# eBay/Sequence-Semantic-Embedding

Measured on AMD Instinct MI355X. Metric: encoded seqs/sec (+ query x target cosine-scores/sec, top-1 vs ref), higher is better.
Workload: dtype f32; 1 GPU; configs[1]: classification stand-in, dual-encoder LSTM H=S=256 E=50 T=32 V=32000; encode 16384 source seqs/GPU/step + cosine top-10 vs 571-target index; batch_per_gpu=16384, seq_len=32, targets=571, parallelism=dp1, weights=random-init (reference initialisers, seed 0)

## Files before the change

### sequence-semantic-embedding_amd/csrc/score_topk.hip

```cpp
#include <cstdlib>

#include "sse_kernels.h"

#define SC_THREADS 512
#define SC_KC 16
#ifndef SC_PRIO_K
#define SC_PRIO_K 1
#define SC_PRIO_E 0
#endif

#ifdef SSE_SCORE_CLOCK
#include <cstdio>
__device__ long long g_score_clk[8 * 8];
#define SC_CLK_DECL long long ck_[8] = {0, 0, 0, 0, 0, 0, 0, 0}, ck_t = clock64();
#define SC_CLK(i)                   \
  {                                 \
    const long long n_ = clock64(); \
    ck_[i] += n_ - ck_t;            \
    ck_t = n_;                      \
  }
#else
#define SC_CLK_DECL
#define SC_CLK(i)
#endif
// ... 786 lines not shown
  hipLaunchKernelGGL(frag32_to_bf16_kernel, dim3((int)(blocks < 16384 ? blocks : 16384)), dim3(256), 0, stream,
                     reinterpret_cast<const f32x4 *>(idxp), NT, KG, KG16, total8, reinterpret_cast<f32x4 *>(out));
  return hipGetLastError();
}

__device__ __forceinline__ int si_key(float f) {
  const int i = __float_as_int(f);
  return i >= 0 ? i : (i ^ 0x7FFFFFFF);
}
__device__ __forceinline__ float si_val(int k) { return __int_as_float(k >= 0 ? k : (k ^ 0x7FFFFFFF)); }
template <int CTRL, int ROWMASK>
__device__ __forceinline__ float dpp_f(float x) {
  return __int_as_float(__builtin_amdgcn_update_dpp(__float_as_int(x), __float_as_int(x), CTRL, ROWMASK, 0xF, false));
}
__device__ __forceinline__ float wave_max_f(float x) {
  x = fmaxf(x, dpp_f<0x128, 0xF>(x));
  x = fmaxf(x, dpp_f<0x124, 0xF>(x));
  x = fmaxf(x, dpp_f<0x122, 0xF>(x));
  x = fmaxf(x, dpp_f<0x121, 0xF>(x));
  x = fmaxf(x, dpp_f<0x142, 0xA>(x));
  x = fmaxf(x, dpp_f<0x143, 0xC>(x));
  return __int_as_float(__builtin_amdgcn_readlane(__float_as_int(x), 63));
}
template <int JMAX>
#ifdef SSE_SCORE_CLOCK
#define SI_CLK_PARAMS , long long (&ck_)[8], long long &ck_t
#define SI_CLK_ARGS , ck_, ck_t
#else
#define SI_CLK_PARAMS
#define SI_CLK_ARGS
#endif
__device__ __forceinline__ void si_select4(const SmallIndexArgs &a, const float *sc, int NP, int NT, int qt, int q0, int lane SI_CLK_PARAMS) {
  constexpr int QW = 4;
  const int J = (NT * 32 + 63) / 64;
  float v[QW][JMAX];
#pragma unroll
  for (int j = 0; j < JMAX; ++j) {
    const int row = lane + 64 * j;
#pragma unroll
    for (int c = 0; c < QW; ++c) v[c][j] = (j < J && row < NT * 32) ? sc[(q0 + c) * NP + row] : NEG_INF;
  }
  int lok[QW], hik[QW];
  float lm[QW];
  bool done[QW];
#pragma unroll
  for (int c = 0; c < QW; ++c) {
    float m = NEG_INF;
#pragma unroll
    for (int j = 0; j < JMAX; ++j) m = fmaxf(m, v[c][j]);
    lm[c] = m;
    lok[c] = si_key(-wave_max_f(-m));
    hik[c] = si_key(wave_max_f(m)) + 1;
    done[c] = false;
  }
  SC_CLK(5)
// ... 23 lines not shown
      int cr = -1, base = 0;
#pragma unroll
      for (int j = 0; j < JMAX; ++j) {
        const bool take = (j < J) & (v[c][j] >= T) & (v[c][j] > NEG_INF);
        const unsigned long long mask = __ballot(take);
        const int n = __popcll(mask);
        const int slot = base + (int)__builtin_amdgcn_mbcnt_hi((unsigned)(mask >> 32), __builtin_amdgcn_mbcnt_lo((unsigned)mask, 0u));
        const int dst = (take && slot < 63) ? slot : 63;
        const int gs = __builtin_amdgcn_ds_permute(dst * 4, __float_as_int(v[c][j]));
        const int gr = __builtin_amdgcn_ds_permute(dst * 4, lane + 64 * j);
        const bool recv = (lane >= base) & (lane < base + n) & (lane < 63);
        cs = recv ? __int_as_float(gs) : cs;
        cr = recv ? gr : cr;
        base += n;
      }
      const int nw = base < 63 ? base : 63;
      int rank = 0;
      for (int l = 0; l < nw; ++l) {
        const float os = __int_as_float(__builtin_amdgcn_readlane(__float_as_int(cs), l));
        const int orow = __builtin_amdgcn_readlane(cr, l);
        rank += ((os > cs) | ((os == cs) & (orow < cr))) ? 1 : 0;
      }
      const bool mine = lane < nw;
      if (mine && rank < SC_KC) {
        a.part_scores[(size_t)query * SC_KC + rank] = cs;
        a.part_ids[(size_t)query * SC_KC + rank] = cr;
      }
      if (lane >= nw && lane < SC_KC) {
        a.part_scores[(size_t)query * SC_KC + lane] = NEG_INF;
        a.part_ids[(size_t)query * SC_KC + lane] = -1;
      }
      const unsigned long long m16 = __ballot(mine && rank == SC_KC - 1);
      const float last = m16 ? __int_as_float(__builtin_amdgcn_readlane(__float_as_int(cs), __ffsll((long long)m16) - 1)) : NEG_INF;
      if (lane == 0) a.part_bnd[query] = (base > 63) ? __builtin_inff() : last;
    }
  }
}

template <int KGC>
__global__ __launch_bounds__(256) void score_small_index_kernel(SmallIndexArgs a) {
  extern __shared__ __attribute__((aligned(16))) float si_sc[];
  const int tid = threadIdx.x, lane = tid & 63, w = __builtin_amdgcn_readfirstlane(tid >> 6);
  const int NT = a.NT, NP = NT * 32 + 1;
  const int qt = blockIdx.x;
  float *sc = si_sc;
  SC_CLK_DECL
  f32x4 b[KGC];
  {
    const int row = qt * 32 + (lane & 31), kb = (lane >> 5) * 4;
    const float *src = a.q_rows + (size_t)(row < a.Q ? row : 0) * a.S + kb;
    const bool vec = (a.S & 3) == 0 && (reinterpret_cast<uintptr_t>(a.q_rows) & 15) == 0 && KGC * 8 <= a.S;
#pragma unroll
    for (int kg = 0; kg < KGC; ++kg) {
      f32x4 v = {0, 0, 0, 0};
      if (vec) {
        v = *reinterpret_cast<const f32x4 *>(src + kg * 8);
      } else {
#pragma unroll
        for (int e = 0; e < 4; ++e)
          if (kg * 8 + kb + e < a.S) v[e] = src[kg * 8 + e];
      }
      if (row >= a.Q) v = f32x4{0, 0, 0, 0};
      b[kg] = v;
    }
  }
  SC_CLK(0)
  for (int t = w; t < NT; t += 4) {
    const f32x4 *ap = reinterpret_cast<const f32x4 *>(a.idxp) + (size_t)t * KGC * 64 + lane;
    f32x16 acc = {0, 0, 0, 0, 0, 0, 0, 0, 0, 0, 0, 0, 0, 0, 0, 0};
    f32x4 ar[4];
#pragma unroll
    for (int d = 0; d < 4; ++d) ar[d] = ap[(d < KGC ? d : 0) * 64];
#pragma unroll
    for (int kg = 0; kg < KGC; ++kg) {
      __builtin_amdgcn_sched_barrier(0);
#pragma unroll
      for (int e = 0; e < 4; ++e) acc = __builtin_amdgcn_mfma_f32_32x32x2f32(ar[kg & 3][e], b[kg][e], acc, 0, 0, 0);
      __builtin_amdgcn_sched_barrier(0);
      ar[kg & 3] = ap[(kg + 4 < KGC ? kg + 4 : kg) * 64];
    }
    const int rb = t * 32 + 4 * (lane >> 5);
    float *col = sc + (lane & 31) * NP;
#pragma unroll
    for (int r = 0; r < 16; ++r) {
      const int row = rb + (r & 3) + 8 * (r >> 2);
      col[row] = (row < a.N) ? acc[r] : NEG_INF;
    }
  }
  SC_CLK(1)
  __syncthreads();
  SC_CLK(2)
  if (NT * 32 <= 640) {
    si_select4<10>(a, sc, NP, NT, qt, w * 8, lane SI_CLK_ARGS);
    SC_CLK(3)
    si_select4<10>(a, sc, NP, NT, qt, w * 8 + 4, lane SI_CLK_ARGS);
    SC_CLK(4)
#ifdef SSE_SCORE_CLOCK
    if (blockIdx.x == gridDim.x / 2 && lane == 0)
      for (int i = 0; i < 8; ++i) g_score_clk[w * 8 + i] = ck_[i];
#endif
  } else {
    si_select4<16>(a, sc, NP, NT, qt, w * 8, lane SI_CLK_ARGS);
    si_select4<16>(a, sc, NP, NT, qt, w * 8 + 4, lane SI_CLK_ARGS);
  }
}
bool score_small_index_applies(int Q, int KG, int64_t NT) {
  return Q >= 1024 && (KG == 32 || KG == 8 || KG == 7) && NT * 32 <= 1024 && (size_t)32 * (NT * 32 + 1) * sizeof(float) <= (size_t)144 * 1024;
}
hipError_t launch_score_small_index(const SmallIndexArgs &a, hipStream_t stream) {
  if (!score_small_index_applies(a.Q, a.KG, a.NT)) return hipErrorInvalidValue;
  const size_t lds = (size_t)32 * (a.NT * 32 + 1) * sizeof(float);
  const dim3 grid((a.Q + 31) / 32), block(256);
  auto go = [&](auto kernel) -> hipError_t {
    hipError_t e = hipFuncSetAttribute(reinterpret_cast<const void *>(kernel), hipFuncAttributeMaxDynamicSharedMemorySize, (int)lds);
    if (e != hipSuccess) return e;
    hipLaunchKernelGGL(kernel, grid, block, lds, stream, a);
    return hipGetLastError();
  };
  if (a.KG == 8) return go(score_small_index_kernel<8>);
  if (a.KG == 7) return go(score_small_index_kernel<7>);
  const hipError_t e32 = go(score_small_index_kernel<32>);
  if (e32 != hipSuccess) return e32;
#ifdef SSE_SCORE_CLOCK
  if (a.Q >= 8192) {
    static int n = 0;
    if (n++ % 8 == 3) {
      long long v[64];
      (void)hipStreamSynchronize(stream);
      (void)hipMemcpyFromSymbol(v, HIP_SYMBOL(g_score_clk), sizeof v);
      for (int w = 0; w < 4; w += 3)
        fprintf(stderr, "[small index clock Q=%d NT=%d] wave %d cycles: query fragments %lld | scores (MFMA + LDS stores) %lld | barrier %lld | selection: loads + bounds %lld | bisection %lld | winners + rank + stores %lld (both batches)\n",
                a.Q, a.NT, w, v[w * 8 + 0], v[w * 8 + 1], v[w * 8 + 2], v[w * 8 + 5], v[w * 8 + 6], v[w * 8 + 3] + v[w * 8 + 4]);
    }
  }
#endif
  return hipGetLastError();
}

hipError_t launch_score_topk(const ScoreArgs &a_in, hipStream_t stream) {
  ScoreArgs a = a_in;
#ifdef SSE_SCORE_MEASURE
  {
    static const int dbg = getenv("SSE_SCORE_DBG") ? atoi(getenv("SSE_SCORE_DBG")) : 0;
    a.dbg = dbg;
// ... 305 lines not shown
      a.cert[qo] = ok ? 1 : 0;
      if (a.col_thr) a.col_thr[qo] = ok ? __builtin_inff() : __double2float_rd(t - (double)(a.eps32 * qnorm));
      if (a.col_slot) {
        a.col_slot[qo] = ok ? -1 : qo;
        a.col_cnt[qo] = 0;
      }
      if (a.host_flag) {
        a.host_cert[qo] = ok ? 1 : 0;
        if (qo == 0 && a.host_err) *a.host_err = a.err_in ? *a.err_in : 0;
        __hip_atomic_store(a.host_flag + qo, a.seq, __ATOMIC_RELEASE, __HIP_MEMORY_SCOPE_SYSTEM);
      }
    }
  }
}

#ifndef RS_NB
#define RS_NB 4
#endif
__device__ __forceinline__ double readlane_f64(double v, int l) {
  const long long b = __double_as_longlong(v);
  const int lo = __builtin_amdgcn_readlane((int)b, l), hi = __builtin_amdgcn_readlane((int)(b >> 32), l);
  return __longlong_as_double(((long long)hi << 32) | (unsigned int)lo);
}
__global__ __launch_bounds__(256) void rescore_small_kernel(RescoreArgs a) {
  const int lane = threadIdx.x & 63;
  const int q = blockIdx.x * 4 + (threadIdx.x >> 6);
  if (q >= a.Q) return;
  if (a.q_count && q >= *a.q_count) return;
  const int qo = a.qmap ? a.qmap[q] : q;
  const float *qrow = a.q + (size_t)q * a.S;
  const int KG = (a.S + 7) / 8;
#ifdef SSE_SCORE_CLOCK
  long long rk_[6] = {0, 0, 0, 0, 0, 0}, rk_t = clock64();
#define RS_CLK(i) { const long long n_ = clock64(); rk_[i] += n_ - rk_t; rk_t = n_; }
#else
#define RS_CLK(i)
#endif
  const bool have = lane < a.NC;
  const int id = have ? a.part_ids[(size_t)q * a.NC + lane] : -1;
  const float sc = have ? a.part_scores[(size_t)q * a.NC + lane] : NEG_INF;
  const float bnd = (lane < a.NC / SC_KC) ? a.part_bnd[(size_t)q * (a.NC / SC_KC) + lane] : NEG_INF;
  double qn = 0.0;
  for (int d = lane; d < a.S; d += 64) qn += (double)qrow[d] * qrow[d];
#pragma unroll
  for (int o = 32; o > 0; o >>= 1) qn += __shfl_xor(qn, o);
  const float qnorm = (float)sqrt(qn);
  const float eps_q = a.eps * qnorm;
  RS_CLK(0)

  unsigned u = __float_as_uint(sc);
  u = (u & 0x80000000u) ? ~u : (u | 0x80000000u);
  const unsigned long long key = (id < 0) ? 0ull : (((unsigned long long)u << 32) | (unsigned long long)(0xFFFFFFFFu - (unsigned)id));
  const int key_lo = (int)(unsigned)key, key_hi = (int)(unsigned)(key >> 32);
  int rank = 0;
  for (int j = 0; j < a.NC; ++j) {
    const unsigned long long kj = ((unsigned long long)(unsigned)__builtin_amdgcn_readlane(key_hi, j) << 32) |
                                  (unsigned long long)(unsigned)__builtin_amdgcn_readlane(key_lo, j);
    rank += (kj > key) ? 1 : 0;
  }
  const unsigned long long kmask = __ballot(key != 0ull && rank == a.k - 1);
  const float kth = kmask ? __int_as_float(__builtin_amdgcn_readlane(__float_as_int(sc), __ffsll((long long)kmask) - 1)) : NEG_INF;
  const bool in_win = (id >= 0) && (sc >= kth - 2.0f * eps_q);
  float mmax = NEG_INF;
  for (int j = 0; j < a.NC / SC_KC; ++j) mmax = fmaxf(mmax, __int_as_float(__builtin_amdgcn_readlane(__float_as_int(bnd), j)));
  const unsigned long long wmask = __ballot(in_win);
  const int nwin = __popcll(wmask);
  const int mi = __popcll(wmask & ((1ull << lane) - 1ull));
  const int idm = __builtin_amdgcn_ds_permute((in_win ? mi : 63) * 4, id);
  RS_CLK(1)
  double exm = -__builtin_inf();
  for (int m0 = 0; m0 < nwin; m0 += RS_NB) {
    int64_t n[RS_NB];
#pragma unroll
    for (int c = 0; c < RS_NB; ++c) n[c] = __builtin_amdgcn_readlane(idm, (m0 + c < nwin) ? m0 + c : 0);
    const double tot = wave_exact_dot_packed<RS_NB>(qrow, a.idx32, a.idx64, n, a.S, KG, lane, a.idx_rm);
    const int want = lane - m0;
    const double got = __shfl(tot, packed_lane_of_value<RS_NB>(want & (RS_NB - 1)));
    if (want >= 0 && want < RS_NB && lane < nwin) exm = got;
  }
  RS_CLK(2)
  int r2 = 0;
  for (int j = 0; j < nwin; ++j)
    r2 += before(readlane_f64(exm, j), (int64_t)__builtin_amdgcn_readlane(idm, j), exm, (int64_t)idm) ? 1 : 0;
  const bool member = lane < nwin;
  if (member && r2 < a.k) {
    a.out_scores[(size_t)qo * a.k + r2] = exm;
    a.out_ids[(size_t)qo * a.k + r2] = a.id_base + idm;
    if (a.host_flag) {
      a.host_scores[(size_t)qo * a.k + r2] = exm;
      a.host_ids[(size_t)qo * a.k + r2] = a.id_base + idm;
    }
  }
  const unsigned long long tmask = __ballot(member && r2 == a.k - 1);
  const double theta = tmask ? readlane_f64(exm, __ffsll((long long)tmask) - 1) : -__builtin_inf();
  if (a.host_flag) __threadfence_system();
  RS_CLK(3)
#ifdef SSE_SCORE_CLOCK
  if (q == a.Q / 2 && lane == 0) {
    rk_[4] = nwin;
    for (int i = 0; i < 6; ++i) g_score_clk[i] = rk_[i];
  }
#endif
  if (lane == 0) {
    const bool ok = (nwin >= a.k) && ((double)mmax + (double)eps_q < theta);
    a.cert[qo] = ok ? 1 : 0;
    if (a.col_thr) a.col_thr[qo] = ok ? __builtin_inff() : __double2float_rd(theta - (double)(a.eps32 * qnorm));
    if (a.col_slot) {
      a.col_slot[qo] = ok ? -1 : qo;
      a.col_cnt[qo] = 0;
    }
    if (a.host_flag) {
      a.host_cert[qo] = ok ? 1 : 0;
      if (qo == 0 && a.host_err) *a.host_err = a.err_in ? *a.err_in : 0;
      __hip_atomic_store(a.host_flag + qo, a.seq, __ATOMIC_RELEASE, __HIP_MEMORY_SCOPE_SYSTEM);
    }
  }
}

hipError_t launch_rescore(const RescoreArgs &a, hipStream_t stream) {
  if (a.NC > RS_MAXNC) return hipErrorInvalidValue;
  if (a.NC <= 64) {
    hipLaunchKernelGGL(rescore_small_kernel, dim3((a.Q + 3) / 4), dim3(256), 0, stream, a);
#ifdef SSE_SCORE_CLOCK
    if (a.Q >= 8192) {
      static int n = 0;
      if (n++ % 8 == 3) {
        long long v[8];
        (void)hipStreamSynchronize(stream);
        (void)hipMemcpyFromSymbol(v, HIP_SYMBOL(g_score_clk), sizeof v);
        fprintf(stderr, "[rescore_small clock Q=%d NC=%d] cycles: query norm %lld | candidates, rank, k-th, window %lld | float64 dots %lld (window of %lld) | exact rank + outputs %lld\n",
                a.Q, a.NC, v[0], v[1], v[2], v[4], v[3]);
      }
    }
#endif
    return hipGetLastError();
  }
  hipLaunchKernelGGL(rescore_kernel, dim3(a.Q), dim3(RS_THREADS), (size_t)a.NC * sizeof(unsigned long long), stream, a);
  return hipGetLastError();
}
// ... 303 lines not shown
```

### sequence-semantic-embedding_amd/csrc/sse_api.hip

```cpp
#include <cmath>
#include <cstdarg>
#include <cstdio>
#include <cstdlib>
#include <algorithm>
#include <chrono>
#include <cstring>
#include <dlfcn.h>
#include <link.h>
#include <mutex>
#include <string>
#include <vector>

#include "../../include/sse_hip.h"
#include "sse_kernels.h"
#include "train.h"

namespace {

thread_local std::string g_create_error;

struct Variable {
  std::string name;
  int rows = 0, cols = 0;
  int64_t count = 0;
// ... 69 lines not shown
};

}

enum { PATH_PERSIST, PATH_CLUSTER, PATH_SMALL, PATH_X3, PATH_GENERIC, PATH_FWD, PATH_FWD_ROWS32, PATH_FWD_ROWS64, PATH_FWD_GS, PATH_FWD_XT,
       PATH_COUNT };
static const char *const LSTM_PATH_NAMES[PATH_COUNT] = {"lstm_path_persist", "lstm_path_cluster", "lstm_path_small", "lstm_path_x3",
                                                "lstm_path_generic", "lstm_path_fwd", "lstm_fwd_rows32", "lstm_fwd_rows64",
                                                "lstm_fwd_gate_split", "lstm_fwd_x_table"};

struct sse_handle {
  sse_config cfg;
  std::mutex mu;
  std::string err;
  std::vector<Variable> vars;
  Encoder enc[2];
  bool packed_dirty = true;
  uint64_t weights_version = 1;
  bool mp_fresh = false;
  bool pad_skip = true;
  int pad_sort_dev = 1;
  int64_t score_two_pass_min_rows = 49152, score_two_pass_rows = 524288;
  int64_t two_pass_calls = 0;
  DevBuf s_lmax;
  bool lstm_gate_split = true;
  DevBuf s_padzero, s_padwork, s_padorder;
  int32_t *pad_stat = nullptr;
  int32_t pad_seq = 0;
  int64_t pad_sorted_calls = 0;
  int64_t lstm_path_calls[10] = {0, 0, 0, 0, 0, 0, 0, 0, 0, 0};
  bool lstm_x3 = false;
  unsigned short *emb16 = nullptr;
  bool emb16_valid = false;
  int lstm_persist_rows = 32;
  uint32_t persist_epoch = 0;
  hipStream_t stream = nullptr;
  bool persist_inject = false;
  int64_t persist_fallbacks = 0;
  int cu_count = 0;
  int lstm_cluster_rows = 1024;
  uint32_t cluster_epoch = 0;
  int lstm_cluster_chunks = 3;
  int cluster_backoff = -1;
  int cluster_skip[2] = {0, 0};
  int lstm_cluster_coop = 1;
  int lstm_cluster_wt = 0;
  int lstm_cluster_drop = 0;
  int lstm_small_rows = 1024;
  int lstm_x_table = 1;
  int lstm_x_table_mb = 256;
  int64_t x_table_builds = 0;
  bool score_small_index = true;
  bool score_bf16 = true;
  void *idxp16 = nullptr;
  size_t idxp16_cap = 0;
  bool idxp16_valid = false;
  bool fb_cnt_init = false;
  bool cnn_bf16 = false;
  unsigned short *emb_bf16 = nullptr, *cnn_Wc16 = nullptr, *cnn_Mx3 = nullptr;
  int lstm_train_rows = 0;
  bool train_bwd_x3 = false;
  bool train_fwd_x3 = false;
  bool train_dk_x3 = false;
  bool train_generic = false;
  bool train_gen1 = false;
  bool train_pair_dedup = true;
  bool train_serial = false;
  float *emb_pad = nullptr;
  int cnn_W[4] = {-1, -1, -1, -1}, cnn_b[4] = {-1, -1, -1, -1}, cnn_M = -1, tgt_table = -1;
  float *cnn_Wc = nullptr, *cnn_bias = nullptr, *cnn_Mp = nullptr;
  int32_t *err_flag = nullptr;
  float *idxp = nullptr;
  size_t idxp_cap = 0;
  double *idx64 = nullptr;
  DevBuf idx_rm;
// ... 874 lines not shown
  if (split) *split = 0;
  if (!h->idxp) return fail(h, "no index uploaded");
  if (Q < 0) return fail(h, "bad Q");
  if (Q == 0) return 0;
  if (k < 1 || k > h->idx_N) return fail(h, "k=%d must be in [1, N=%lld]", k, (long long)h->idx_N);
  if ((k > 16) && phase == SCORE_REST) return 0;
  if (k > SSE_MAX_SELECT_K) {
    HIPCHECK(h, launch_exact_topk(q, h->idxp, h->idx64, nullptr, out_s, out_i, h->idx_base, h->idx_N, Q, h->idx_S, k, st));
    return 0;
  }
  if (k > 16) return score_select_locked(h, q, Q, k, out_s, out_i, st);
  const int S = h->idx_S, KG = (S + 7) / 8;
  const int QT = (Q + 31) / 32;
  const bool bf = h->score_bf16 && h->idx_N >= 8192;
  const int NQ = score_pick_nq(Q, S, bf ? 1 : 0);
  if (NQ == 0) return fail(h, "index dimension %d does not fit the scoring kernel's LDS query block", S);
  const int QB = (QT + NQ - 1) / NQ;
  const int64_t NT = (h->idx_N + 31) / 32;
  const int nsplit = choose_nsplit(NQ, QB, NT);
  int nsplit2 = nsplit;
  static const int split2_max = getenv("SSE_SPLIT2_MAX") ? atoi(getenv("SSE_SPLIT2_MAX")) : 128;
  while (nsplit2 < split2_max && NT / (nsplit2 * 2 * 2) >= 16) nsplit2 *= 2;
  const bool small_idx = h->score_small_index && !bf && score_small_index_applies(Q, KG, NT);
  const int NC = small_idx ? 16 : nsplit * 16, NCmax = std::max(nsplit, nsplit2) * 16;
  const int KG16 = (S + 15) / 16;
  if (bf && !h->idxp16_valid) {
    const size_t need = (size_t)NT * KG16 * 1024;
    if (need > h->idxp16_cap) {
      if (h->idxp16) HIPCHECK(h, hipFree(h->idxp16));
      h->idxp16 = nullptr;
      h->idxp16_cap = 0;
      HIPCHECK(h, hipMalloc(&h->idxp16, need));
      h->idxp16_cap = need;
    }
    HIPCHECK(h, launch_frag32_to_bf16(h->idxp, NT, KG, h->idxp16, st));
    h->idxp16_valid = true;
  }
  if (ensure_counters(h, st)) return 1;
  unsigned long long *counters = (unsigned long long *)h->s_fb_cnt.p;
  if (bf && NQ == 4 && Q >= 1024 && h->idx_N >= h->score_two_pass_min_rows && h->idx_N <= h->score_two_pass_rows && !mirror) {
    int ns2 = std::min(nsplit, 16);
    {
      static const int force = getenv("SSE_TWO_PASS_SPLITS") ? atoi(getenv("SSE_TWO_PASS_SPLITS")) : 0;
      const int cus = h->cu_count > 0 ? h->cu_count : 256;
      double best = 0.0;
      for (int ns = 1; ns <= 16; ns *= 2) {
// ... 30 lines not shown
    m1.KG = KG16;
    m1.NT = (int)NT;
    m1.QT = QT;
    m1.NSPLIT = ns2;
    m1.KC = 16;
    m1.NQ = NQ;
    m1.lane_max = (float *)h->s_lmax.p;
    HIPCHECK(h, launch_score_topk(m1, st));
    HIPCHECK(h, launch_lane_max_threshold(q, (const float *)h->s_lmax.p, Q, S, ns2 * 16, eps_bf, (float *)h->s_cthr.p,
                                          (int32_t *)h->s_cslot.p, st));
    ScoreArgs m2 = m1;
    m2.lane_max = nullptr;
    m2.col_thr = (const float *)h->s_cthr.p;
    m2.col_slot = (const int32_t *)h->s_cslot.p;
    m2.col_cnt = (int32_t *)h->s_ccnt.p;
    m2.col_buf = (int32_t *)h->s_cbuf.p;
    m2.col_cap = MID_CAP;
    HIPCHECK(h, launch_score_topk(m2, st));
    SelectArgs sel{q, h->idxp, h->idx64, m2.col_slot, m2.col_cnt, m2.col_buf, MID_CAP, out_s, out_i, (int32_t *)h->s_cert.p, h->idx_base,
                   Q, S, k, nullptr};
    HIPCHECK(h, launch_select_topk(sel, st));
    HIPCHECK(h, launch_exact_topk(q, h->idxp, h->idx64, (const int32_t *)h->s_cert.p, out_s, out_i, h->idx_base, h->idx_N, Q, S, k, st,
                                  counters + 2));
    if (split) *split = 0;
    return 0;
  }
  const int POOL = std::min(Q, 1024);
  if (reserve(h, h->s_qp, (size_t)QB * NQ * KG * 256 * sizeof(float))) return 1;
  if (reserve(h, h->s_ps, (size_t)Q * (bf ? NCmax : NC) * sizeof(float))) return 1;
  if (reserve(h, h->s_pi, (size_t)Q * (bf ? NCmax : NC) * sizeof(int32_t))) return 1;
  if (reserve(h, h->s_pb, (size_t)Q * (bf ? NCmax / 16 : nsplit) * sizeof(float))) return 1;
  if (reserve(h, h->s_cert, (size_t)Q * sizeof(int32_t))) return 1;
  if (reserve_collect(h, Q, POOL)) return 1;
  if (split) *split = 1;
  const bool first = phase != SCORE_REST, rest = phase != SCORE_FIRST;
  const bool rows_direct = NQ == 1;
  if (first && !rows_direct && !small_idx) {
    if (bf) HIPCHECK(h, launch_pack_rows_bf16(q, Q, S, h->s_qp.p, st));
    else HIPCHECK(h, launch_pack_rows(q, Q, S, (float *)h->s_qp.p, st));
  }
  ScoreArgs a;
  if (rows_direct) {
    a.q_rows = q;
    a.S = S;
  }
  a.BF = bf ? 1 : 0;
// ... 485 lines not shown
  if (bits) {
    if (check_err_flag(h, nullptr, &bits)) return 1;
    if (bits == 4) {
      if (encode_fallback_locked(h, side, B, T, normalize, nullptr)) return 1;
      if (score_to_host_locked(h, (const float *)h->s_out.p, B, k, out_scores, out_ids)) return 1;
    }
  }
  if (enc_out_host)
    HIPCHECK(h, hipMemcpy(enc_out_host, h->s_out.p, (size_t)B * h->cfg.encoding_size * sizeof(float), hipMemcpyDeviceToHost));
  return 0;
}

int sse_get_counter(sse_handle *h, const char *name, int64_t *value) {
  if (!h || !name || !value) return 1;
  std::lock_guard<std::mutex> lk(h->mu);
  if (strcmp(name, "lstm_persist_fallbacks") == 0) {
    *value = h->persist_fallbacks;
    return 0;
  }
  if (strcmp(name, "score_two_pass_calls") == 0) {
    *value = h->two_pass_calls;
    return 0;
  }
  if (strcmp(name, "pad_sorted_calls") == 0) {
    *value = h->pad_sorted_calls;
    return 0;
  }
  if (strcmp(name, "lstm_x_table_builds") == 0) {
    *value = h->x_table_builds;
    return 0;
  }
  for (int i = 0; i < PATH_COUNT; ++i) {
    if (strcmp(name, LSTM_PATH_NAMES[i]) != 0) continue;
    *value = h->lstm_path_calls[i];
    return 0;
  }
  if (strcmp(name, "lstm_coop_refused") == 0) {
    *value = (int64_t)lstm_coop_refused();
    return 0;
  }
  static const char *const names[3] = {"score_bf16_second_chance_queries", "score_collect_queries", "score_bruteforce_queries"};
  for (int i = 0; i < 3; ++i) {
    if (strcmp(name, names[i]) != 0) continue;
    unsigned long long v[4] = {0, 0, 0, 0};
    if (h->s_fb_cnt.p && h->fb_cnt_init) {
      HIPCHECK(h, hipSetDevice(h->cfg.device));
      HIPCHECK(h, hipDeviceSynchronize());
      HIPCHECK(h, hipMemcpy(v, h->s_fb_cnt.p, sizeof v, hipMemcpyDeviceToHost));
    }
    *value = (int64_t)v[i];
    return 0;
  }
  return fail(h, "unknown counter '%s'", name);
}

int sse_set_option(sse_handle *h, const char *name, int32_t value) {
  if (!h || !name) return 1;
  std::lock_guard<std::mutex> lk(h->mu);
  if (strcmp(name, "score_small_index") == 0) {
    h->score_small_index = value != 0;
    return 0;
  }
  if (strcmp(name, "score_bf16") == 0) {
    h->score_bf16 = value != 0;
    return 0;
  }
  if (strcmp(name, "cnn_bf16") == 0) {
    if (h->cfg.network_mode != SSE_MODE_SOURCE_ONLY_CNN) return fail(h, "option cnn_bf16 needs network_mode source_only_cnn");
    h->cnn_bf16 = value != 0;
    h->packed_dirty = true;
    h->mp_fresh = false;
    return 0;
  }
  if (strcmp(name, "lstm_train_rows") == 0) {
    if (value != 0 && value != 32 && value != 64) return fail(h, "lstm_train_rows must be 0, 32 or 64");
    h->lstm_train_rows = (int)value;
    return 0;
  }
  if (strcmp(name, "train_bwd_x3") == 0) {
    h->train_bwd_x3 = value != 0;
    return 0;
  }
  if (strcmp(name, "train_fwd_x3") == 0) {
// ... 1127 lines not shown
```

### sequence-semantic-embedding_amd/csrc/sse_kernels.h

```cpp
#pragma once
#include <hip/hip_runtime.h>
#include <stdint.h>

typedef float f32x4 __attribute__((ext_vector_type(4)));
typedef float f32x16 __attribute__((ext_vector_type(16)));

__host__ __device__ static inline int frag32_off(int r_in_tile, int k_in_group) {
  return ((((k_in_group >> 2) << 5) + r_in_tile) << 2) + (k_in_group & 3);
}

__device__ static inline int mfma_row(int reg, int lane) { return (reg & 3) + 8 * (reg >> 2) + 4 * (lane >> 5); }

static inline int round_up(int x, int m) { return (x + m - 1) / m * m; }

typedef unsigned int sse_u32x4 __attribute__((ext_vector_type(4)));
__host__ __device__ static inline unsigned short sse_bf16_rne(float f) {
  unsigned u;
  __builtin_memcpy(&u, &f, 4);
  u += 0x7FFFu + ((u >> 16) & 1u);
  return (unsigned short)(u >> 16);
}
__host__ __device__ static inline float sse_bf16_f32(unsigned short h) {
  const unsigned u = (unsigned)h << 16;
  float f;
// ... 246 lines not shown
  float *col_thr = nullptr;
  float eps32 = 0.0f;
  int32_t *col_slot = nullptr, *col_cnt = nullptr;
  double *host_scores = nullptr;
  int64_t *host_ids = nullptr;
  int32_t *host_cert = nullptr, *host_flag = nullptr, *host_err = nullptr;
  const int32_t *err_in = nullptr;
  int32_t seq = 0;
  const float *idx_rm = nullptr;
};
hipError_t launch_rescore(const RescoreArgs &a, hipStream_t stream);

struct SmallIndexArgs {
  const float *q_rows;
  const float *idxp;
  float *part_scores;
  int32_t *part_ids;
  float *part_bnd;
  int64_t N;
  int32_t Q, S, KG, NT;
};
bool score_small_index_applies(int Q, int KG, int64_t NT);
hipError_t launch_score_small_index(const SmallIndexArgs &a, hipStream_t stream);

hipError_t launch_assign_slots(const int32_t *cert, int Q, int slots, int32_t *col_slot, int32_t *counter, hipStream_t st);
hipError_t launch_kth_bound(const float *q, const float *part_scores, const int32_t *part_ids, int Q, int S, int NC, int k,
                            float eps, float *col_thr, int32_t *col_slot, hipStream_t st);
struct SelectArgs {
  const float *q;
  const float *idx32;
  const double *idx64;
  const int32_t *col_slot, *col_cnt, *col_buf;
  int32_t col_cap;
  double *out_scores;
  int64_t *out_ids;
  int32_t *cert;
  int64_t id_base;
  int32_t Q, S, k;
  unsigned long long *served = nullptr;
};
hipError_t launch_select_topk(const SelectArgs &a, hipStream_t st);

hipError_t launch_merge_topk(const double *in_s, const int64_t *in_i, int64_t stride, int P, int Q, int k, double *out_s,
                             int64_t *out_i, hipStream_t stream);

hipError_t launch_pack_rows(const float *rows, int64_t R, int C, float *out, hipStream_t stream);
// ... 56 lines not shown
```

Baseline: 7.466 million seqs/s.

## Fuse small-index scoring, float64 rescoring and fallback into one kernel

Adds a fused small-index kernel that computes cosine scores into LDS, selects per-query candidates in registers, runs the float64 certification in the same wave, and serves uncertified queries from the LDS score row without further launches. This removes the partial-result round trip through global memory and the separate rescore, select and exact-topk launches. It also caches the hipFuncSetAttribute call per device and kernel. The cost is more register and code pressure in one kernel, plus serial per-query fallback work inside the block. The scoring step is a small part of the encode-plus-score workload.

```diff
diff --git a/sequence-semantic-embedding_amd/csrc/score_topk.hip b/sequence-semantic-embedding_amd/csrc/score_topk.hip
--- a/sequence-semantic-embedding_amd/csrc/score_topk.hip
+++ b/sequence-semantic-embedding_amd/csrc/score_topk.hip
@@ -1,3 +1,4 @@
+#include <atomic>
 #include <cstdlib>
 
 #include "sse_kernels.h"
@@ -832,7 +833,7 @@
   x = fmaxf(x, dpp_f<0x143, 0xC>(x));
   return __int_as_float(__builtin_amdgcn_readlane(__float_as_int(x), 63));
 }
-template <int JMAX>
+template <int JMAX, bool FUSED>
 #ifdef SSE_SCORE_CLOCK
 #define SI_CLK_PARAMS , long long (&ck_)[8], long long &ck_t
 #define SI_CLK_ARGS , ck_, ck_t
@@ -840,7 +841,8 @@
 #define SI_CLK_PARAMS
 #define SI_CLK_ARGS
 #endif
-__device__ __forceinline__ void si_select4(const SmallIndexArgs &a, const float *sc, int NP, int NT, int qt, int q0, int lane SI_CLK_PARAMS) {
+__device__ __forceinline__ void si_select4(const SmallIndexArgs &a, const float *sc, int NP, int NT, int qt, int q0, int lane,
+                                           float (&ws)[4], int (&wr)[4], float (&wb)[4] SI_CLK_PARAMS) {
   constexpr int QW = 4;
   const int J = (NT * 32 + 63) / 64;
   float v[QW][JMAX];
@@ -910,19 +912,76 @@
         rank += ((os > cs) | ((os == cs) & (orow < cr))) ? 1 : 0;
       }
       const bool mine = lane < nw;
-      if (mine && rank < SC_KC) {
-        a.part_scores[(size_t)query * SC_KC + rank] = cs;
-        a.part_ids[(size_t)query * SC_KC + rank] = cr;
-      }
-      if (lane >= nw && lane < SC_KC) {
-        a.part_scores[(size_t)query * SC_KC + lane] = NEG_INF;
-        a.part_ids[(size_t)query * SC_KC + lane] = -1;
-      }
       const unsigned long long m16 = __ballot(mine && rank == SC_KC - 1);
       const float last = m16 ? __int_as_float(__builtin_amdgcn_readlane(__float_as_int(cs), __ffsll((long long)m16) - 1)) : NEG_INF;
-      if (lane == 0) a.part_bnd[query] = (base > 63) ? __builtin_inff() : last;
-    }
-  }
+      if constexpr (FUSED) {
+        const int dst = (mine && rank < SC_KC) ? rank : 63;
+        const int gs = __builtin_amdgcn_ds_permute(dst * 4, __float_as_int(cs));
+        const int gr = __builtin_amdgcn_ds_permute(dst * 4, cr);
+        const bool got = lane < (nw < SC_KC ? nw : SC_KC);
+        ws[c] = got ? __int_as_float(gs) : NEG_INF;
+        wr[c] = got ? gr : -1;
+        wb[c] = (base > 63) ? __builtin_inff() : last;
+      } else {
+        if (mine && rank < SC_KC) {
+          a.part_scores[(size_t)query * SC_KC + rank] = cs;
+          a.part_ids[(size_t)query * SC_KC + rank] = cr;
+        }
+        if (lane >= nw && lane < SC_KC) {
+          a.part_scores[(size_t)query * SC_KC + lane] = NEG_INF;
+          a.part_ids[(size_t)query * SC_KC + lane] = -1;
+        }
+        if (lane == 0) a.part_bnd[query] = (base > 63) ? __builtin_inff() : last;
+      }
+    }
+  }
+}
+
+template <int KGC>
+__device__ __forceinline__ void si_scores_to_lds(const SmallIndexArgs &a, float *sc, int NT, int NP, int qt, int lane, int w SI_CLK_PARAMS) {
+  f32x4 b[KGC];
+  {
+    const int row = qt * 32 + (lane & 31), kb = (lane >> 5) * 4;
+    const float *src = a.q_rows + (size_t)(row < a.Q ? row : 0) * a.S + kb;
+    const bool vec = (a.S & 3) == 0 && (reinterpret_cast<uintptr_t>(a.q_rows) & 15) == 0 && KGC * 8 <= a.S;
+#pragma unroll
+    for (int kg = 0; kg < KGC; ++kg) {
+      f32x4 v = {0, 0, 0, 0};
+      if (vec) {
+        v = *reinterpret_cast<const f32x4 *>(src + kg * 8);
+      } else {
+#pragma unroll
+        for (int e = 0; e < 4; ++e)
+          if (kg * 8 + kb + e < a.S) v[e] = src[kg * 8 + e];
+      }
+      if (row >= a.Q) v = f32x4{0, 0, 0, 0};
+      b[kg] = v;
+    }
+  }
+  SC_CLK(0)
+  for (int t = w; t < NT; t += 4) {
+    const f32x4 *ap = reinterpret_cast<const f32x4 *>(a.idxp) + (size_t)t * KGC * 64 + lane;
+    f32x16 acc = {0, 0, 0, 0, 0, 0, 0, 0, 0, 0, 0, 0, 0, 0, 0, 0};
+    f32x4 ar[4];
+#pragma unroll
+    for (int d = 0; d < 4; ++d) ar[d] = ap[(d < KGC ? d : 0) * 64];
+#pragma unroll
+    for (int kg = 0; kg < KGC; ++kg) {
+      __builtin_amdgcn_sched_barrier(0);
+#pragma unroll
+      for (int e = 0; e < 4; ++e) acc = __builtin_amdgcn_mfma_f32_32x32x2f32(ar[kg & 3][e], b[kg][e], acc, 0, 0, 0);
+      __builtin_amdgcn_sched_barrier(0);
+      ar[kg & 3] = ap[(kg + 4 < KGC ? kg + 4 : kg) * 64];
+    }
+    const int rb = t * 32 + 4 * (lane >> 5);
+    float *col = sc + (lane & 31) * NP;
+#pragma unroll
+    for (int r = 0; r < 16; ++r) {
+      const int row = rb + (r & 3) + 8 * (r >> 2);
+      col[row] = (row < a.N) ? acc[r] : NEG_INF;
+    }
+  }
+  SC_CLK(1)
 }
 
 template <int KGC>
@@ -933,81 +992,49 @@
   const int qt = blockIdx.x;
   float *sc = si_sc;
   SC_CLK_DECL
-  f32x4 b[KGC];
-  {
-    const int row = qt * 32 + (lane & 31), kb = (lane >> 5) * 4;
-    const float *src = a.q_rows + (size_t)(row < a.Q ? row : 0) * a.S + kb;
-    const bool vec = (a.S & 3) == 0 && (reinterpret_cast<uintptr_t>(a.q_rows) & 15) == 0 && KGC * 8 <= a.S;
-#pragma unroll
-    for (int kg = 0; kg < KGC; ++kg) {
-      f32x4 v = {0, 0, 0, 0};
-      if (vec) {
-        v = *reinterpret_cast<const f32x4 *>(src + kg * 8);
-      } else {
-#pragma unroll
-        for (int e = 0; e < 4; ++e)
-          if (kg * 8 + kb + e < a.S) v[e] = src[kg * 8 + e];
-      }
-      if (row >= a.Q) v = f32x4{0, 0, 0, 0};
-      b[kg] = v;
-    }
-  }
-  SC_CLK(0)
-  for (int t = w; t < NT; t += 4) {
-    const f32x4 *ap = reinterpret_cast<const f32x4 *>(a.idxp) + (size_t)t * KGC * 64 + lane;
-    f32x16 acc = {0, 0, 0, 0, 0, 0, 0, 0, 0, 0, 0, 0, 0, 0, 0, 0};
-    f32x4 ar[4];
-#pragma unroll
-    for (int d = 0; d < 4; ++d) ar[d] = ap[(d < KGC ? d : 0) * 64];
-#pragma unroll
-    for (int kg = 0; kg < KGC; ++kg) {
-      __builtin_amdgcn_sched_barrier(0);
-#pragma unroll
-      for (int e = 0; e < 4; ++e) acc = __builtin_amdgcn_mfma_f32_32x32x2f32(ar[kg & 3][e], b[kg][e], acc, 0, 0, 0);
-      __builtin_amdgcn_sched_barrier(0);
-      ar[kg & 3] = ap[(kg + 4 < KGC ? kg + 4 : kg) * 64];
-    }
-    const int rb = t * 32 + 4 * (lane >> 5);
-    float *col = sc + (lane & 31) * NP;
-#pragma unroll
-    for (int r = 0; r < 16; ++r) {
-      const int row = rb + (r & 3) + 8 * (r >> 2);
-      col[row] = (row < a.N) ? acc[r] : NEG_INF;
-    }
-  }
-  SC_CLK(1)
+  si_scores_to_lds<KGC>(a, sc, NT, NP, qt, lane, w SI_CLK_ARGS);
   __syncthreads();
   SC_CLK(2)
+  float ws[4], wb[4];
+  int wr[4];
   if (NT * 32 <= 640) {
-    si_select4<10>(a, sc, NP, NT, qt, w * 8, lane SI_CLK_ARGS);
+    si_select4<10, false>(a, sc, NP, NT, qt, w * 8, lane, ws, wr, wb SI_CLK_ARGS);
     SC_CLK(3)
-    si_select4<10>(a, sc, NP, NT, qt, w * 8 + 4, lane SI_CLK_ARGS);
+    si_select4<10, false>(a, sc, NP, NT, qt, w * 8 + 4, lane, ws, wr, wb SI_CLK_ARGS);
     SC_CLK(4)
 #ifdef SSE_SCORE_CLOCK
     if (blockIdx.x == gridDim.x / 2 && lane == 0)
       for (int i = 0; i < 8; ++i) g_score_clk[w * 8 + i] = ck_[i];
 #endif
   } else {
-    si_select4<16>(a, sc, NP, NT, qt, w * 8, lane SI_CLK_ARGS);
-    si_select4<16>(a, sc, NP, NT, qt, w * 8 + 4, lane SI_CLK_ARGS);
+    si_select4<16, false>(a, sc, NP, NT, qt, w * 8, lane, ws, wr, wb SI_CLK_ARGS);
+    si_select4<16, false>(a, sc, NP, NT, qt, w * 8 + 4, lane, ws, wr, wb SI_CLK_ARGS);
   }
 }
 bool score_small_index_applies(int Q, int KG, int64_t NT) {
   return Q >= 1024 && (KG == 32 || KG == 8 || KG == 7) && NT * 32 <= 1024 && (size_t)32 * (NT * 32 + 1) * sizeof(float) <= (size_t)144 * 1024;
+}
+template <class K, class A>
+static hipError_t si_launch(K kernel, int slot, size_t lds, dim3 grid, hipStream_t stream, const A &args) {
+  static std::atomic<unsigned char> raised[6][64];
+  int dev = 0;
+  hipError_t e = hipGetDevice(&dev);
+  if (e != hipSuccess) return e;
+  if (dev < 0 || dev >= 64 || !raised[slot][dev].load(std::memory_order_acquire)) {
+    e = hipFuncSetAttribute(reinterpret_cast<const void *>(kernel), hipFuncAttributeMaxDynamicSharedMemorySize, 144 * 1024);
+    if (e != hipSuccess) return e;
+    if (dev >= 0 && dev < 64) raised[slot][dev].store(1, std::memory_order_release);
+  }
+  hipLaunchKernelGGL(kernel, grid, dim3(256), lds, stream, args);
+  return hipGetLastError();
 }
 hipError_t launch_score_small_index(const SmallIndexArgs &a, hipStream_t stream) {
   if (!score_small_index_applies(a.Q, a.KG, a.NT)) return hipErrorInvalidValue;
   const size_t lds = (size_t)32 * (a.NT * 32 + 1) * sizeof(float);
-  const dim3 grid((a.Q + 31) / 32), block(256);
-  auto go = [&](auto kernel) -> hipError_t {
-    hipError_t e = hipFuncSetAttribute(reinterpret_cast<const void *>(kernel), hipFuncAttributeMaxDynamicSharedMemorySize, (int)lds);
-    if (e != hipSuccess) return e;
-    hipLaunchKernelGGL(kernel, grid, block, lds, stream, a);
-    return hipGetLastError();
-  };
-  if (a.KG == 8) return go(score_small_index_kernel<8>);
-  if (a.KG == 7) return go(score_small_index_kernel<7>);
-  const hipError_t e32 = go(score_small_index_kernel<32>);
+  const dim3 grid((a.Q + 31) / 32);
+  if (a.KG == 8) return si_launch(score_small_index_kernel<8>, 0, lds, grid, stream, a);
+  if (a.KG == 7) return si_launch(score_small_index_kernel<7>, 1, lds, grid, stream, a);
+  const hipError_t e32 = si_launch(score_small_index_kernel<32>, 2, lds, grid, stream, a);
   if (e32 != hipSuccess) return e32;
 #ifdef SSE_SCORE_CLOCK
   if (a.Q >= 8192) {
@@ -1359,24 +1386,18 @@
   const int lo = __builtin_amdgcn_readlane((int)b, l), hi = __builtin_amdgcn_readlane((int)(b >> 32), l);
   return __longlong_as_double(((long long)hi << 32) | (unsigned int)lo);
 }
-__global__ __launch_bounds__(256) void rescore_small_kernel(RescoreArgs a) {
-  const int lane = threadIdx.x & 63;
-  const int q = blockIdx.x * 4 + (threadIdx.x >> 6);
-  if (q >= a.Q) return;
-  if (a.q_count && q >= *a.q_count) return;
-  const int qo = a.qmap ? a.qmap[q] : q;
-  const float *qrow = a.q + (size_t)q * a.S;
-  const int KG = (a.S + 7) / 8;
 #ifdef SSE_SCORE_CLOCK
-  long long rk_[6] = {0, 0, 0, 0, 0, 0}, rk_t = clock64();
+#define RS_CLK_PARAMS , long long (&rk_)[6], long long &rk_t
+#define RS_CLK_ARGS , rk_, rk_t
 #define RS_CLK(i) { const long long n_ = clock64(); rk_[i] += n_ - rk_t; rk_t = n_; }
 #else
+#define RS_CLK_PARAMS
+#define RS_CLK_ARGS
 #define RS_CLK(i)
 #endif
-  const bool have = lane < a.NC;
-  const int id = have ? a.part_ids[(size_t)q * a.NC + lane] : -1;
-  const float sc = have ? a.part_scores[(size_t)q * a.NC + lane] : NEG_INF;
-  const float bnd = (lane < a.NC / SC_KC) ? a.part_bnd[(size_t)q * (a.NC / SC_KC) + lane] : NEG_INF;
+__device__ __forceinline__ bool rescore_small_wave(const RescoreArgs &a, const float *qrow, int qo, int NC, int id, float sc, float mmax,
+                                                   int lane, double &theta_out, float &qnorm_out RS_CLK_PARAMS) {
+  const int KG = (a.S + 7) / 8;
   double qn = 0.0;
   for (int d = lane; d < a.S; d += 64) qn += (double)qrow[d] * qrow[d];
 #pragma unroll
@@ -1390,7 +1411,7 @@
   const unsigned long long key = (id < 0) ? 0ull : (((unsigned long long)u << 32) | (unsigned long long)(0xFFFFFFFFu - (unsigned)id));
   const int key_lo = (int)(unsigned)key, key_hi = (int)(unsigned)(key >> 32);
   int rank = 0;
-  for (int j = 0; j < a.NC; ++j) {
+  for (int j = 0; j < NC; ++j) {
     const unsigned long long kj = ((unsigned long long)(unsigned)__builtin_amdgcn_readlane(key_hi, j) << 32) |
                                   (unsigned long long)(unsigned)__builtin_amdgcn_readlane(key_lo, j);
     rank += (kj > key) ? 1 : 0;
@@ -1398,8 +1419,6 @@
   const unsigned long long kmask = __ballot(key != 0ull && rank == a.k - 1);
   const float kth = kmask ? __int_as_float(__builtin_amdgcn_readlane(__float_as_int(sc), __ffsll((long long)kmask) - 1)) : NEG_INF;
   const bool in_win = (id >= 0) && (sc >= kth - 2.0f * eps_q);
-  float mmax = NEG_INF;
-  for (int j = 0; j < a.NC / SC_KC; ++j) mmax = fmaxf(mmax, __int_as_float(__builtin_amdgcn_readlane(__float_as_int(bnd), j)));
   const unsigned long long wmask = __ballot(in_win);
   const int nwin = __popcll(wmask);
   const int mi = __popcll(wmask & ((1ull << lane) - 1ull));
@@ -1433,13 +1452,38 @@
   if (a.host_flag) __threadfence_system();
   RS_CLK(3)
 #ifdef SSE_SCORE_CLOCK
+  rk_[4] = nwin;
+#endif
+  theta_out = theta;
+  qnorm_out = qnorm;
+  return (nwin >= a.k) && ((double)mmax + (double)eps_q < theta);
+}
+
+__global__ __launch_bounds__(256) void rescore_small_kernel(RescoreArgs a) {
+  const int lane = threadIdx.x & 63;
+  const int q = blockIdx.x * 4 + (threadIdx.x >> 6);
+  if (q >= a.Q) return;
+  if (a.q_count && q >= *a.q_count) return;
+  const int qo = a.qmap ? a.qmap[q] : q;
+  const float *qrow = a.q + (size_t)q * a.S;
+#ifdef SSE_SCORE_CLOCK
+  long long rk_[6] = {0, 0, 0, 0, 0, 0}, rk_t = clock64();
+#endif
+  const bool have = lane < a.NC;
+  const int id = have ? a.part_ids[(size_t)q * a.NC + lane] : -1;
+  const float sc = have ? a.part_scores[(size_t)q * a.NC + lane] : NEG_INF;
+  const float bnd = (lane < a.NC / SC_KC) ? a.part_bnd[(size_t)q * (a.NC / SC_KC) + lane] : NEG_INF;
+  float mmax = NEG_INF;
+  for (int j = 0; j < a.NC / SC_KC; ++j) mmax = fmaxf(mmax, __int_as_float(__builtin_amdgcn_readlane(__float_as_int(bnd), j)));
+  double theta;
+  float qnorm;
+  const bool ok = rescore_small_wave(a, qrow, qo, a.NC, id, sc, mmax, lane, theta, qnorm RS_CLK_ARGS);
+#ifdef SSE_SCORE_CLOCK
   if (q == a.Q / 2 && lane == 0) {
-    rk_[4] = nwin;
     for (int i = 0; i < 6; ++i) g_score_clk[i] = rk_[i];
   }
 #endif
   if (lane == 0) {
-    const bool ok = (nwin >= a.k) && ((double)mmax + (double)eps_q < theta);
     a.cert[qo] = ok ? 1 : 0;
     if (a.col_thr) a.col_thr[qo] = ok ? __builtin_inff() : __double2float_rd(theta - (double)(a.eps32 * qnorm));
     if (a.col_slot) {
@@ -1452,6 +1496,140 @@
       __hip_atomic_store(a.host_flag + qo, a.seq, __ATOMIC_RELEASE, __HIP_MEMORY_SCOPE_SYSTEM);
     }
   }
+}
+
+__device__ __forceinline__ void si_serve_uncertified(const RescoreArgs &a, const float *srow, int nrows, const float *qrow, int query,
+                                                     double theta, float qnorm, int lane, unsigned long long *served) {
+  const int KG = (a.S + 7) / 8;
+  float thr = __double2float_rd(theta - (double)(a.eps32 * qnorm));
+  int reach = 0;
+  for (int j0 = 0; j0 < nrows; j0 += 64) {
+    const float s = (j0 + lane < nrows) ? srow[j0 + lane] : NEG_INF;
+    reach += __popcll(__ballot(s >= thr && s > NEG_INF));
+  }
+  if (reach < a.k) thr = NEG_INF;
+  double ls = -__builtin_inf();
+  int lr = 0x7FFFFFFF;
+  for (int j0 = 0; j0 < nrows; j0 += 64) {
+    const float s = (j0 + lane < nrows) ? srow[j0 + lane] : NEG_INF;
+    unsigned long long mask = __ballot(s >= thr && s > NEG_INF);
+    while (mask) {
+      int64_t n[RS_NB];
+      int cnt = 0;
+      const int first = j0 + __ffsll((long long)mask) - 1;
+#pragma unroll
+      for (int c = 0; c < RS_NB; ++c) {
+        n[c] = mask ? j0 + __ffsll((long long)mask) - 1 : first;
+        cnt += mask ? 1 : 0;
+        mask &= mask - 1ull;
+      }
+      const double tot = wave_exact_dot_packed<RS_NB>(qrow, a.idx32, a.idx64, n, a.S, KG, lane, a.idx_rm);
+#pragma unroll
+      for (int c = 0; c < RS_NB; ++c) {
+        if (c < cnt) {
+          const double s64 = readlane_f64(tot, packed_lane_of_value<RS_NB>(c));
+          const int p = __popcll(__ballot(before(ls, (int64_t)lr, s64, n[c])));
+          const double us = __shfl_up(ls, 1);
+          const int ur = __shfl_up(lr, 1);
+          if (lane == p) {
+            ls = s64;
+            lr = (int)n[c];
+          } else if (lane > p) {
+            ls = us;
+            lr = ur;
+          }
+        }
+      }
+    }
+  }
+  if (lane < a.k) {
+    a.out_scores[(size_t)query * a.k + lane] = ls;
+    a.out_ids[(size_t)query * a.k + lane] = a.id_base + lr;
+  }
+  if (lane == 0 && served) atomicAdd(served, 1ull);
+}
+
+template <int JMAX>
+__device__ __forceinline__ void si_fused_rank(const SmallIndexFusedArgs &f, const float *sc, int NP, int NT, int qt, int w, int lane SI_CLK_PARAMS) {
+  const SmallIndexArgs &a = f.s;
+#ifdef SSE_SCORE_CLOCK
+  long long rk_[6] = {0, 0, 0, 0, 0, 0}, rk_t = 0;
+#endif
+#pragma unroll 1
+  for (int half = 0; half < 2; ++half) {
+    const int q0 = w * 8 + half * 4;
+    float ws[4], wb[4];
+    int wr[4];
+#pragma unroll
+    for (int c = 0; c < 4; ++c) {
+      ws[c] = NEG_INF;
+      wb[c] = NEG_INF;
+      wr[c] = -1;
+    }
+    si_select4<JMAX, true>(a, sc, NP, NT, qt, q0, lane, ws, wr, wb SI_CLK_ARGS);
+    SC_CLK(3)
+#pragma unroll 1
+    for (int c = 0; c < 4; ++c) {
+      const int query = qt * 32 + q0 + c;
+      if (query >= a.Q) break;
+      const float s = c == 0 ? ws[0] : c == 1 ? ws[1] : c == 2 ? ws[2] : ws[3];
+      const int id = c == 0 ? wr[0] : c == 1 ? wr[1] : c == 2 ? wr[2] : wr[3];
+      const float bnd = c == 0 ? wb[0] : c == 1 ? wb[1] : c == 2 ? wb[2] : wb[3];
+      const float *qrow = a.q_rows + (size_t)query * a.S;
+      double theta;
+      float qnorm;
+      const bool ok = rescore_small_wave(f.r, qrow, query, SC_KC, id, s, bnd, lane, theta, qnorm RS_CLK_ARGS);
+      if (!ok) si_serve_uncertified(f.r, sc + (q0 + c) * NP, NT * 32, qrow, query, theta, qnorm, lane, f.served);
+      if (lane == 0) f.r.cert[query] = 1;
+    }
+    SC_CLK(7)
+  }
+}
+
+template <int KGC>
+__global__ __launch_bounds__(256) void score_small_index_fused_kernel(SmallIndexFusedArgs f) {
+  extern __shared__ __attribute__((aligned(16))) float si_sc[];
+  const int tid = threadIdx.x, lane = tid & 63, w = __builtin_amdgcn_readfirstlane(tid >> 6);
+  const int NT = f.s.NT, NP = NT * 32 + 1;
+  const int qt = blockIdx.x;
+  float *sc = si_sc;
+  SC_CLK_DECL
+  si_scores_to_lds<KGC>(f.s, sc, NT, NP, qt, lane, w SI_CLK_ARGS);
+  __syncthreads();
+  SC_CLK(2)
+  if (NT * 32 <= 640) si_fused_rank<10>(f, sc, NP, NT, qt, w, lane SI_CLK_ARGS);
+  else si_fused_rank<16>(f, sc, NP, NT, qt, w, lane SI_CLK_ARGS);
+#ifdef SSE_SCORE_CLOCK
+  if (blockIdx.x == gridDim.x / 2 && lane == 0)
+    for (int i = 0; i < 8; ++i) g_score_clk[w * 8 + i] = ck_[i];
+#endif
+}
+
+hipError_t launch_score_small_index_fused(const SmallIndexFusedArgs &f, hipStream_t stream) {
+  const SmallIndexArgs &a = f.s;
+  if (!score_small_index_applies(a.Q, a.KG, a.NT)) return hipErrorInvalidValue;
+  if (f.r.k < 1 || f.r.k > SC_KC || f.r.host_flag || f.r.qmap || f.r.q_count || f.r.q != a.q_rows) return hipErrorInvalidValue;
+  const size_t lds = (size_t)32 * (a.NT * 32 + 1) * sizeof(float);
+  const dim3 grid((a.Q + 31) / 32);
+  hipError_t e;
+  if (a.KG == 8) e = si_launch(score_small_index_fused_kernel<8>, 3, lds, grid, stream, f);
+  else if (a.KG == 7) e = si_launch(score_small_index_fused_kernel<7>, 4, lds, grid, stream, f);
+  else e = si_launch(score_small_index_fused_kernel<32>, 5, lds, grid, stream, f);
+  if (e != hipSuccess) return e;
+#ifdef SSE_SCORE_CLOCK
+  if (a.Q >= 8192 && a.KG == 32) {
+    static int n = 0;
+    if (n++ % 8 == 3) {
+      long long v[64];
+      (void)hipStreamSynchronize(stream);
+      (void)hipMemcpyFromSymbol(v, HIP_SYMBOL(g_score_clk), sizeof v);
+      for (int w = 0; w < 4; w += 3)
+        fprintf(stderr, "[small index fused clock Q=%d NT=%d] wave %d cycles: query fragments %lld | scores (MFMA + LDS stores) %lld | barrier %lld | selection: loads + bounds %lld | bisection %lld | winners + rank + permute %lld | float64 ranking %lld (both batches)\n",
+                a.Q, a.NT, w, v[w * 8 + 0], v[w * 8 + 1], v[w * 8 + 2], v[w * 8 + 5], v[w * 8 + 6], v[w * 8 + 3], v[w * 8 + 7]);
+    }
+  }
+#endif
+  return hipGetLastError();
 }
 
 hipError_t launch_rescore(const RescoreArgs &a, hipStream_t stream) {
diff --git a/sequence-semantic-embedding_amd/csrc/sse_api.hip b/sequence-semantic-embedding_amd/csrc/sse_api.hip
--- a/sequence-semantic-embedding_amd/csrc/sse_api.hip
+++ b/sequence-semantic-embedding_amd/csrc/sse_api.hip
@@ -115,6 +115,7 @@
   int pad_sort_dev = 1;
   int64_t score_two_pass_min_rows = 49152, score_two_pass_rows = 524288;
   int64_t two_pass_calls = 0;
+  int64_t fused_calls = 0;
   DevBuf s_lmax;
   bool lstm_gate_split = true;
   DevBuf s_padzero, s_padwork, s_padorder;
@@ -143,7 +144,7 @@
   int lstm_x_table = 1;
   int lstm_x_table_mb = 256;
   int64_t x_table_builds = 0;
-  bool score_small_index = true;
+  int score_small_index = 1;
   bool score_bf16 = true;
   void *idxp16 = nullptr;
   size_t idxp16_cap = 0;
@@ -1064,6 +1065,7 @@
   static const int split2_max = getenv("SSE_SPLIT2_MAX") ? atoi(getenv("SSE_SPLIT2_MAX")) : 128;
   while (nsplit2 < split2_max && NT / (nsplit2 * 2 * 2) >= 16) nsplit2 *= 2;
   const bool small_idx = h->score_small_index && !bf && score_small_index_applies(Q, KG, NT);
+  const bool small_fused = small_idx && h->score_small_index == 1 && !mirror;
   const int NC = small_idx ? 16 : nsplit * 16, NCmax = std::max(nsplit, nsplit2) * 16;
   const int KG16 = (S + 15) / 16;
   if (bf && !h->idxp16_valid) {
@@ -1140,6 +1142,36 @@
     HIPCHECK(h, launch_select_topk(sel, st));
     HIPCHECK(h, launch_exact_topk(q, h->idxp, h->idx64, (const int32_t *)h->s_cert.p, out_s, out_i, h->idx_base, h->idx_N, Q, S, k, st,
                                   counters + 2));
+    if (split) *split = 0;
+    return 0;
+  }
+  if (small_fused) {
+    if (phase == SCORE_REST) return 0;
+    h->fused_calls += 1;
+    if (reserve(h, h->s_cert, (size_t)Q * sizeof(int32_t))) return 1;
+    const float eps32 = (float)(2.0 * (S + 2) * 5.97e-8 * h->idx_norm_max);
+    SmallIndexFusedArgs f;
+    f.s = SmallIndexArgs{q, h->idxp, nullptr, nullptr, nullptr, h->idx_N, Q, S, KG, (int)NT};
+    f.r.q = q;
+    f.r.idx32 = h->idxp;
+    f.r.idx64 = h->idx64;
+    f.r.idx_rm = h->idx_rm_valid ? (const float *)h->idx_rm.p : nullptr;
+    f.r.part_scores = nullptr;
+    f.r.part_ids = nullptr;
+    f.r.part_bnd = nullptr;
+    f.r.out_scores = out_s;
+    f.r.out_ids = out_i;
+    f.r.cert = (int32_t *)h->s_cert.p;
+    f.r.id_base = h->idx_base;
+    f.r.N = h->idx_N;
+    f.r.Q = Q;
+    f.r.S = S;
+    f.r.NC = 16;
+    f.r.k = k;
+    f.r.eps = eps32;
+    f.r.eps32 = eps32;
+    f.served = counters + 1;
+    HIPCHECK(h, launch_score_small_index_fused(f, st));
     if (split) *split = 0;
     return 0;
   }
@@ -1671,6 +1703,10 @@
     *value = h->two_pass_calls;
     return 0;
   }
+  if (strcmp(name, "score_fused_calls") == 0) {
+    *value = h->fused_calls;
+    return 0;
+  }
   if (strcmp(name, "pad_sorted_calls") == 0) {
     *value = h->pad_sorted_calls;
     return 0;
@@ -1707,7 +1743,8 @@
   if (!h || !name) return 1;
   std::lock_guard<std::mutex> lk(h->mu);
   if (strcmp(name, "score_small_index") == 0) {
-    h->score_small_index = value != 0;
+    if (value < 0 || value > 2) return fail(h, "option score_small_index takes 0 (list sweep), 1 (fused launch) or 2 (two kernels)");
+    h->score_small_index = value;
     return 0;
   }
   if (strcmp(name, "score_bf16") == 0) {
diff --git a/sequence-semantic-embedding_amd/csrc/sse_kernels.h b/sequence-semantic-embedding_amd/csrc/sse_kernels.h
--- a/sequence-semantic-embedding_amd/csrc/sse_kernels.h
+++ b/sequence-semantic-embedding_amd/csrc/sse_kernels.h
@@ -292,6 +292,12 @@
 };
 bool score_small_index_applies(int Q, int KG, int64_t NT);
 hipError_t launch_score_small_index(const SmallIndexArgs &a, hipStream_t stream);
+struct SmallIndexFusedArgs {
+  SmallIndexArgs s;
+  RescoreArgs r;
+  unsigned long long *served;
+};
+hipError_t launch_score_small_index_fused(const SmallIndexFusedArgs &f, hipStream_t stream);
 
 hipError_t launch_assign_slots(const int32_t *cert, int Q, int slots, int32_t *col_slot, int32_t *counter, hipStream_t st);
 hipError_t launch_kth_bound(const float *q, const float *part_scores, const int32_t *part_ids, int Q, int S, int NC, int k,
```

Result: no change. 7.489 million seqs/s (median of 6 runs) (+0.3%).
